# worxli/ORB_SLAM

Hardware: AMD Instinct MI355X
Metric: frames/sec ORB extract+match (640x480, 1000 kp) (higher is better)
Workload: dtype u8

## Files before the change

### orb_slam_amd/__init__.py

```python
import ctypes
import os
from pathlib import Path

import numpy as np

_PKG = Path(__file__).resolve().parent
LIB_PATH = Path(os.environ.get("ORBX_LIBRARY", _PKG / "liborbx.so"))

ORBX_OK = 0
ERRORS = {-1: "ORBX_ERR_ARG", -2: "ORBX_ERR_HIP", -3: "ORBX_ERR_CAPACITY",
          -4: "ORBX_ERR_UNSUPPORTED", -5: "ORBX_ERR_NOMEM", -6: "ORBX_ERR_NOT_POSDEF"}

KEYPOINT = np.dtype([("x", "<f4"), ("y", "<f4"), ("size", "<f4"), ("angle", "<f4"),
                     ("response", "<f4"), ("octave", "<i4"), ("class_id", "<i4")])
assert KEYPOINT.itemsize == 28


class OrbxError(RuntimeError):
    def __init__(self, code, where):
        super().__init__(f"{where}: {ERRORS.get(code, code)}")
        self.code = code


class FrameView(ctypes.Structure):
# ... 505 lines not shown
        "orbx_dev_search_by_projection_frame_kf": ([vp, i, vp, i, vp, vp, vp, vp, vp, f, i, i, vp, i, ip], i),
        "orbx_dev_search_by_sim3": ([vp, i, vp, i, vp, vp, vp, vp, vp, vp, vp, vp, f, vp, vp, f, vp, vp, i, ip], i),
        "orbx_search_by_sim3": ([vp, vp, vp, vp, vp, vp, vp, vp, vp, vp, f, vp, vp, f, vp, vp, ip], i),
        "orbx_distinctive_descriptors": ([vp, i, vp, vp, vp], i),
        "orbx_search_by_projection_kf_sim3": ([vp, vp, vp, vp, vp, vp, i, vp, ip], i),
        "orbx_search_by_projection_frame_kf": ([vp, vp, vp, vp, vp, vp, vp, vp, f, i, i, vp, ip], i),
        "orbx_vocab_create": ([vp, i, i, i, vp, vp, vp, vp, ctypes.POINTER(vp)], i),
        "orbx_vocab_destroy": ([vp], None),
        "orbx_vocab_n_words": ([vp], i),
        "orbx_vocab_transform": ([vp, vp, i, vp, i, vp, vp, vp, vp, vp, ip, vp, vp, vp, ip], i),
        "orbx_dev_compute_bow": ([vp, vp, i, i, i], i),
        "orbx_dev_read_bow": ([vp, i, i, vp, vp, vp, vp, vp, ip, vp, vp, vp, ip], i),
        "orbx_dev_search_by_bow": ([vp, i, i, vp, f, i, vp, i, vp], i),
        "orbx_dev_search_by_bow_kf": ([vp, i, vp, i, vp, vp, f, i, vp, i, vp], i),
        "orbx_dev_search_for_triangulation": ([vp, i, vp, i, vp, vp, vp, vp, i, i, vp, i, vp], i),
        "orbx_undistort_keypoints": ([vp, i, vp, vp, vp, vp], i),
        "orbx_compute_image_bounds": ([i, i, vp, vp, vp], i),
        "orbx_dev_undistort": ([vp, i, i, vp, vp], i),
        "orbx_pose_optimization": ([vp, vp, ip, vp], i),
        "orbx_pose_optimization_batch": ([vp, i, vp, vp, vp], i),
        "orbx_pose_stage": ([vp, i, vp], i),
        "orbx_pose_run": ([vp], i),
        "orbx_pose_fetch": ([vp, vp, vp, vp], i),
        "orbx_version": ([], ctypes.c_char_p),
        "orbx_abi_version": ([], i),
        "orbx_lba_set_workgroups": ([vp, i], i),
        "orbx_lba_get_workgroups": ([vp], i),
        "orbx_lba_last_workgroups": ([vp], i),
        "orbx_debug_lba_split": ([vp, i, i, i, i], i),
        "orbx_debug_describe_patch": ([vp, i, i, i, i, vp], i),
        "orbx_debug_level0_direct": ([vp], i),
        "orbx_debug_fast_instance": ([vp, vp], i),
        "orbx_debug_fast_lists": ([vp, i, vp, i, vp, i, vp], i),
        "orbx_pose_set_exact": ([vp, i], i),
        "orbx_pose_get_exact": ([vp], i),
        "orbx_dev_set_image_bounds": ([vp, vp], i),
        "orbx_set_launch_mode": ([vp, i], i),
        "orbx_get_launch_mode": ([vp], i),
        "orbx_host_alloc": ([sz, ctypes.POINTER(vp)], i),
        "orbx_host_free": ([vp], None),
        "orbx_dev_upload_async": ([vp, i, i, vp, i, i, sz], i),
        "orbx_dev_download_async": ([vp, i, i, vp, vp, vp, vp, vp], i),
        "orbx_describe_levels": ([i, f, i, i, i, i, vp, i], i),
        "orbx_init_models": ([vp, vp], i),
        "orbx_init_models_batch": ([vp, i, vp], i),
        "orbx_dev_init_models": ([vp, i, i, i, f, i, vp], i),
        "orbx_dev_read_init_models": ([vp, i, vp], i),
        "orbx_init_reconstruct": ([vp, vp], i),
        "orbx_init_reconstruct_batch": ([vp, i, vp], i),
        "orbx_dev_init_reconstruct": ([vp, i, i, i, vp, f, f, i], i),
        "orbx_dev_read_init_reconstruct": ([vp, i, vp, ip], i),
        "orbx_triangulate_matches": ([vp, vp, i, vp, i, vp, vp, vp, vp, vp, vp, vp, vp], i),
        "orbx_create_new_map_points": ([vp, vp, vp, i, vp, vp, vp, i, i, vp, vp, vp, vp, vp, vp], i),
        "orbx_dev_create_new_map_points": ([vp, i, vp, vp, i, vp, vp, vp, vp, i, i, vp, vp, vp, vp, vp, vp, i], i),
        "orbx_sim3_ransac": ([vp, vp], i),
        "orbx_sim3_ransac_batch": ([vp, i, vp], i),
        "orbx_pnp_ransac": ([vp, vp], i),
        "orbx_pnp_ransac_batch": ([vp, i, vp], i),
        "orbx_dev_pnp_candidates": ([vp, i, i, vp, vp, vp, vp, i, f, i, i, vp, i, vp, vp, vp], i),
        "orbx_dev_sim3_candidates": ([vp, i, vp, i, vp, vp, f, i, i, ctypes.c_double, i, i, i, vp, vp, i, vp, vp, vp], i),
        "orbx_optimize_sim3": ([vp, vp], i),
        "orbx_optimize_sim3_batch": ([vp, i, vp], i),
        "orbx_dev_optimize_sim3": ([vp, i, vp, vp, i, vp, vp, vp], i),
    }
    for name, (args, res) in sigs.items():
        fn = getattr(L, name)
# ... 144 lines not shown
                                            ctypes.byref(n)), "orbx_dev_read_features")
        return kps[:n.value].copy(), desc[:n.value].copy()

    def matches(self, slot):
        m = np.zeros(self.nfeatures, np.int32)
        nm, n1 = ctypes.c_int(0), ctypes.c_int(0)
        _check(lib().orbx_dev_read_matches(self._h, slot, _ptr(m), self.nfeatures, ctypes.byref(nm),
                                           ctypes.byref(n1)), "orbx_dev_read_matches")
        return m, nm.value

    def level(self, slot, level, blurred=False, cap=4 << 20):
        buf = np.zeros(cap, np.uint8)
        pw, ph = ctypes.c_int(0), ctypes.c_int(0)
        _check(lib().orbx_dev_read_level(self._h, slot, level, int(blurred), _ptr(buf), cap,
                                         ctypes.byref(pw), ctypes.byref(ph)), "orbx_dev_read_level")
        return buf[:pw.value * ph.value].reshape(ph.value, pw.value).copy()

    def describe_patch(self, slot, level, x, y):
        out = np.zeros((37, 37), np.uint8)
        _check(lib().orbx_debug_describe_patch(self._h, slot, level, x, y, _ptr(out)), "orbx_debug_describe_patch")
        return out

    def level0_direct(self):
        r = lib().orbx_debug_level0_direct(self._h)
        if r < 0:
            raise OrbxError(r, "orbx_debug_level0_direct")
        return bool(r)

    def fast_instance(self):
        out = np.zeros(3, np.int32)
        _check(lib().orbx_debug_fast_instance(self._h, _ptr(out)), "orbx_debug_fast_instance")
        return tuple(int(v) for v in out)

    def fast_lists(self, slot, cells_cap=1 << 14, lists_cap=1 << 22):
        cells = np.zeros(10 * cells_cap, np.int32)
        lists = np.zeros(lists_cap, np.uint32)
        ne = ctypes.c_int(0)
        n = lib().orbx_debug_fast_lists(self._h, slot, _ptr(cells), cells.size, _ptr(lists), lists.size,
                                        ctypes.byref(ne))
        _check(min(n, 0), "orbx_debug_fast_lists")
        out = []
        for level, ini_x, ini_y, hx, hy, valid, off, cap, cnt, _ in cells[:10 * n].reshape(n, 10):
            assert 0 <= cnt <= cap and off + cnt <= ne.value, (cnt, cap, off, ne.value)
            e = lists[off:off + cnt]
            xy = np.stack([e & 0xFFF, (e >> 12) & 0xFFF, e >> 24], axis=1).astype(np.int64)
            out.append((int(level), int(ini_x), int(ini_y), int(hx), int(hy), bool(valid), xy))
        return out

    def timing(self, enable=True, only=None):
        _check(lib().orbx_dev_kernel_time_select(self._h, only.encode() if only else None), "timing")
        _check(lib().orbx_dev_kernel_time_enable(self._h, int(enable)), "timing")

    def kernel_time(self, name):
        avg, tot = ctypes.c_double(0), ctypes.c_double(0)
        n = lib().orbx_dev_kernel_time(self._h, name.encode(), ctypes.byref(avg), ctypes.byref(tot))
        if n < 0:
            raise OrbxError(n, "orbx_dev_kernel_time")
        return n, avg.value, tot.value

    def pose_optimization(self, frames):
        from .synth_pose import PoseStats
        arr = (type(frames[0]) * len(frames))(*frames)
        n = np.zeros(len(frames), np.int32)
        st = (PoseStats * len(frames))()
        _check(lib().orbx_pose_optimization_batch(self._h, len(frames), arr, _ptr(n), st),
               "orbx_pose_optimization_batch")
# ... 356 lines not shown
```

### orb_slam_amd/csrc/orbx_api.cpp

```cpp
#include <cstdlib>
#include <algorithm>
#include <cstring>
#include <new>

#include "orbx_internal.h"

using namespace orbx;

namespace orbx {

static KernelTimer* find_timer(orbx_ctx* ctx, const char* name)
{
    for (auto& t : ctx->timers)
        if (t.name == name) return &t;
    ctx->timers.push_back(KernelTimer{name, {}, {}, 0});
    return &ctx->timers.back();
}

void timer_begin(orbx_ctx* ctx, const char* name, hipStream_t st)
{
    if (!ctx->timing || (!ctx->timing_only.empty() && ctx->timing_only != name)) return;
    KernelTimer* t = find_timer(ctx, name);
    if (t->used == (int)t->start.size()) {
        hipEvent_t a, b;
// ... 21 lines not shown
    ctx->scratch_bytes = 0;
    if (hipMalloc(&ctx->scratch, bytes) != hipSuccess) return ORBX_ERR_NOMEM;
    ctx->scratch_bytes = bytes;
    return ORBX_OK;
}

int ensure_pinned(orbx_ctx* ctx, size_t bytes)
{
    if (bytes <= ctx->host_pinned_bytes) return ORBX_OK;
    if (ctx->host_pinned) hipHostFree(ctx->host_pinned);
    ctx->host_pinned = nullptr;
    ctx->host_pinned_bytes = 0;
    if (hipHostMalloc(&ctx->host_pinned, bytes, hipHostMallocDefault) != hipSuccess) return ORBX_ERR_NOMEM;
    ctx->host_pinned_bytes = bytes;
    return ORBX_OK;
}

template <typename T>
static int realloc_dev(T*& p, size_t count)
{
    if (p) (void)hipFree(p);
    p = nullptr;
    if (count == 0) count = 1;
    if (hipMalloc(reinterpret_cast<void**>(&p), count * sizeof(T)) != hipSuccess) return ORBX_ERR_NOMEM;
    return ORBX_OK;
}

static void free_buffers(orbx_ctx* ctx)
{
    void* ptrs[] = {ctx->frames, ctx->pyr_raw, ctx->pyr_blur, ctx->cell_lists, ctx->retain_scratch, ctx->cell_count,
                    ctx->level_keys, ctx->cell_keys64, ctx->level_keys64, ctx->level_count, ctx->out_kps, ctx->out_desc, ctx->out_n,
                    ctx->match12, ctx->match_n, ctx->error_flags, ctx->dgeom.levels, ctx->dgeom.cells,
                    ctx->dgeom.res_cols, ctx->dgeom.res_rows, ctx->dgeom.umax, ctx->blur_tiles, ctx->cascade,
                    ctx->scratch, ctx->pose_dev, ctx->bow_dev};
    for (void* p : ptrs)
        if (p) (void)hipFree(p);
    if (ctx->host_pinned) (void)hipHostFree(ctx->host_pinned);
    if (ctx->pose_host) (void)hipHostFree(ctx->pose_host);
}

static int set_geometry(orbx_ctx* ctx, int w, int h)
{
    if (ctx->geom_w == w && ctx->geom_h == h) return ORBX_OK;
    if (w > ctx->max_w || h > ctx->max_h) return ORBX_ERR_CAPACITY;
    hipStreamSynchronize(ctx->stream);
    Geometry& g = ctx->geom;
    int r = compute_geometry(g, w, h);
    if (r != ORBX_OK) return r;
    plan_cascade(g, kCascadeLds);
    const int S = ctx->slots;
    if ((long long)w * h > (long long)ctx->cap_frame_px) {
        if ((r = realloc_dev(ctx->frames, (size_t)S * w * h)) != ORBX_OK) return r;
        ctx->cap_frame_px = (long long)w * h;
    }
    if (g.frame_pyr_bytes > ctx->cap_pyr_bytes) {
        if ((r = realloc_dev(ctx->pyr_raw, (size_t)S * g.frame_pyr_bytes)) != ORBX_OK) return r;
        if ((r = realloc_dev(ctx->pyr_blur, (size_t)g.frame_pyr_bytes)) != ORBX_OK) return r;
        ctx->cap_pyr_bytes = g.frame_pyr_bytes;
    }
    if (g.list_entries + 4LL * (long long)g.cells.size() > ctx->cap_list_entries) {
        const long long e = g.list_entries + 4LL * (long long)g.cells.size();
        if ((r = realloc_dev(ctx->cell_lists, (size_t)S * e)) != ORBX_OK) return r;
        if ((r = realloc_dev(ctx->retain_scratch, (size_t)S * e)) != ORBX_OK) return r;
        if (ctx->harris && (r = realloc_dev(ctx->cell_keys64, (size_t)S * e)) != ORBX_OK) return r;
        ctx->cap_list_entries = e;
    }
    if ((int)g.cells.size() > ctx->cap_cells) {
        if ((r = realloc_dev(ctx->cell_count, (size_t)S * g.cells.size())) != ORBX_OK) return r;
        if ((r = realloc_dev(ctx->dgeom.cells, g.cells.size())) != ORBX_OK) return r;
        ctx->cap_cells = (int)g.cells.size();
    }
    if (g.level_entries > ctx->cap_level_entries) {
        if ((r = realloc_dev(ctx->level_keys, (size_t)S * g.level_entries)) != ORBX_OK) return r;
        if (ctx->harris && (r = realloc_dev(ctx->level_keys64, (size_t)S * g.level_entries)) != ORBX_OK) return r;
        ctx->cap_level_entries = g.level_entries;
    }
    if ((int)g.res_cols.size() > ctx->cap_res_cols) {
        if ((r = realloc_dev(ctx->dgeom.res_cols, g.res_cols.size())) != ORBX_OK) return r;
        ctx->cap_res_cols = (int)g.res_cols.size();
    }
    if ((int)g.res_rows.size() > ctx->cap_res_rows) {
        if ((r = realloc_dev(ctx->dgeom.res_rows, g.res_rows.size())) != ORBX_OK) return r;
        ctx->cap_res_rows = (int)g.res_rows.size();
    }
    std::vector<int4> tiles;
    for (int l = 0; l < g.nlevels; l++) {
        const LevelGeom& L = g.levels[l];
        const int ndw = L.stride / 4, nstrips = (L.ph + kBlurStrip - 1) / kBlurStrip;
        const int nchunks = (ndw + kBlurChunkCols - 1) / kBlurChunkCols;
        for (int b = 0; b < nchunks * nstrips; b += kBlurItems / 64) tiles.push_back(make_int4(l, b, nchunks, nstrips));
    }
    if ((int)tiles.size() > ctx->cap_blur_tiles) {
        if ((r = realloc_dev(ctx->blur_tiles, tiles.size())) != ORBX_OK) return r;
        ctx->cap_blur_tiles = (int)tiles.size();
    }
    ctx->blur_tiles_n = (int)tiles.size();
    ORBX_HIP_CHECK(hipMemcpy(ctx->dgeom.levels, g.levels.data(), g.levels.size() * sizeof(LevelGeom), hipMemcpyHostToDevice));
    ORBX_HIP_CHECK(hipMemcpy(ctx->dgeom.cells, g.cells.data(), g.cells.size() * sizeof(CellGeom), hipMemcpyHostToDevice));
    if (!g.res_cols.empty())
        ORBX_HIP_CHECK(hipMemcpy(ctx->dgeom.res_cols, g.res_cols.data(), g.res_cols.size() * sizeof(ResizeCol), hipMemcpyHostToDevice));
    if (!g.res_rows.empty())
// ... 659 lines not shown
```

### orb_slam_amd/csrc/orbx_extract.hip

```cpp
#include <algorithm>
#include <type_traits>

#include "orbx_device.h"
#include "orbx_internal.h"

namespace orbx {

constexpr size_t kRetainLds = 128 * 1024;
constexpr int kRetainCellCap = 512;
constexpr int kSplitMinFrames = 16;
constexpr size_t kResizeLds = 96 * 1024;

__constant__ __attribute__((aligned(4))) int8_t c_pattern[256][4] = {
#include "orbx_pattern.inc"
};

#ifdef ORBX_FAST_PROFILE
__device__ unsigned long long g_fast_prof[24];
__device__ inline unsigned long long fp_stamp()
{
    unsigned long long t;
    asm volatile("s_memtime %0\n\ts_waitcnt lgkmcnt(0)" : "=s"(t)::"memory");
    return t;
}
#define FP_T0() unsigned long long _ft = fp_stamp()
#define FP_MARK(k)                                                                  \
    do {                                                                            \
        const unsigned long long _n = fp_stamp();                                   \
        if (threadIdx.x == 0) atomicAdd(&g_fast_prof[k], _n - _ft);                 \
        _ft = _n;                                                                   \
    } while (0)
#define FP_ADD(k, v) atomicAdd(&g_fast_prof[k], (unsigned long long)(v))
extern "C" int orbx_debug_fast_prof(unsigned long long* out)
{
    return hipMemcpyFromSymbol(out, HIP_SYMBOL(g_fast_prof), sizeof(unsigned long long) * 24) == hipSuccess ? 0 : -2;
}
#else
#define FP_T0()
#define FP_MARK(k)
#define FP_ADD(k, v)
#endif

struct ExtractArgs {
    const LevelGeom* levels;
    const CellGeom* cells;
    const ResizeCol* res_cols;
    const ResizeRow* res_rows;
    const int* umax;
    const uint8_t* frames;
    uint8_t* pyr_raw;
    uint8_t* pyr_blur;
    uint32_t* cell_lists;
    int32_t* cell_count;
    uint32_t* level_keys;
    int32_t* level_count;
    orbx_keypoint* out_kps;
    uint8_t* out_desc;
    int32_t* out_n;
    int32_t* error_flags;
    uint8_t* host_out;
    int32_t* retain_scratch;
    uint64_t* cell_keys64;
    uint64_t* level_keys64;
    int harris;
    int fp_contract;
    int nth_pivot;
    long long frame_pyr_bytes;
    int first_slot;
    int w, h;
    int nlevels, ncells, list_entries, level_entries, nfeatures;
    int fast_th, fast_th_low;
    int max_list_cap, max_level_cap;
    int l0_direct;
};

struct LevelSrc {
    const uint8_t* base;
    int stride;
};
static_assert(kEdge % 16 == 0, "the direct level 0 keeps the padded level's 16-byte alignment");
__device__ __forceinline__ LevelSrc level_src(const ExtractArgs& a, int f, int level, long long off, int stride)
{
    if (a.l0_direct && level == 0)
        return {a.frames + ((long long)(a.first_slot + f) * a.w * a.h - (long long)kEdge * a.w - kEdge), a.w};
    return {a.pyr_raw + (size_t)f * a.frame_pyr_bytes + off, stride};
}
// ... 612 lines not shown
                       __builtin_elementwise_minimum(e0, e9));
    }
    orbx_h2 dk = h2_max3(m[0], m[1], m[2]), br = h2_min3(x[0], x[1], x[2]);
    dk = h2_max3(dk, m[3], m[4]);
    br = h2_min3(br, x[3], x[4]);
    dk = h2_max3(dk, m[5], m[6]);
    br = h2_min3(br, x[5], x[6]);
    dk = __builtin_elementwise_maximum(dk, m[7]);
    br = __builtin_elementwise_minimum(br, x[7]);
    return __builtin_bit_cast(uint32_t, __builtin_elementwise_maximum(dk, -br));
}

__device__ inline int byte_of(uint32_t w, int k) { return (int)((w >> (8 * k)) & 0xFF); }

typedef short orbx_s16x2 __attribute__((ext_vector_type(2)));
__device__ inline uint32_t pk_sub16(uint32_t a, uint32_t b)
{
    return __builtin_bit_cast(uint32_t, (orbx_s16x2)(__builtin_bit_cast(orbx_s16x2, a) - __builtin_bit_cast(orbx_s16x2, b)));
}
__device__ inline uint32_t pk_max16(uint32_t a, uint32_t b)
{
    return __builtin_bit_cast(uint32_t,
                              __builtin_elementwise_max(__builtin_bit_cast(orbx_s16x2, a), __builtin_bit_cast(orbx_s16x2, b)));
}
__device__ inline orbx_h2 h2_bytes(uint32_t w, uint32_t k64, uint32_t sel)
{
    return __builtin_bit_cast(orbx_h2, __builtin_amdgcn_perm(k64, w, sel));
}

constexpr int kFastWideThreads = 256;
__host__ __device__ constexpr int fast_tile_bytes(int hy_max, int pitch) { return (hy_max * pitch + 511) & ~511; }
__host__ __device__ constexpr int fast_lds_bytes(int tile_bytes) { return 2 * tile_bytes + tile_bytes / 32; }
__host__ __device__ constexpr int fast_static_lds(bool u32_entries) { return 4 * 384 * (u32_entries ? 4 : 2) + 64; }
#ifndef ORBX_FAST_LDS_TARGET
#define ORBX_FAST_LDS_TARGET (40 * 1024)
#endif
constexpr int kFastLdsTarget = ORBX_FAST_LDS_TARGET;
#ifndef ORBX_DIAG_REPEAT
#define ORBX_DIAG_REPEAT 1, 1, 1, 1
#endif
constexpr int kDiagRepeat[4] = {ORBX_DIAG_REPEAT};

template <int kP, int kThreads = 256, bool kBanded = false>
__global__ __launch_bounds__(kThreads) __attribute__((amdgpu_waves_per_eu(kThreads > 256 ? 6 : 4))) void k_fast_cells(
    ExtractArgs a, int tile_bytes, int band_rows)
{
    constexpr int kBlock = kThreads, kWaves = kThreads / 64;
    extern __shared__ __attribute__((aligned(16))) uint8_t smem[];
    __shared__ BlockScratchN<kWaves> bs;
    using QEntry = typename std::conditional<kP != 0, uint16_t, uint32_t>::type;
    constexpr int kQueue = 128 + 256;
    constexpr int kQueueWords = kWaves * kQueue * (int)sizeof(QEntry) / 4;
    constexpr int kUnitCap = 2 * kQueueWords;
    __shared__ __attribute__((aligned(16))) uint32_t qbuf[kQueueWords];
    __shared__ int s_left[kWaves];
    uint16_t* ulist = reinterpret_cast<uint16_t*>(qbuf);
    const int f = blockIdx.y, tid = threadIdx.x, lane = tid & 63, wv = tid >> 6;
    QEntry* cand = reinterpret_cast<QEntry*>(qbuf) + wv * kQueue;
    const int clear16 = (tile_bytes + tile_bytes / 32) >> 4;
    auto clear_maps_at = [&](uint8_t* sm) {
        for (int i = tid; i < clear16; i += kBlock) reinterpret_cast<uint4*>(sm)[i] = make_uint4(0, 0, 0, 0);
    };
    auto process = [&](const int cell, uint8_t* const tile, uint8_t* const sm) {
    const CellGeom C = cget(a.cells, cell);
    int32_t* count_out = a.cell_count + (size_t)f * a.ncells + cell;
    if (!C.valid) {
        if (tid == 0) *count_out = 0;
        return;
    }
    const LevelGeom L = cget(a.levels, C.level);
    const int roi_x = kEdge + C.ini_x, x_al = roi_x & ~15, sh = roi_x - x_al;
    const int hx = C.hx, hy = C.hy;
    const int nq16 = (sh + hx + 15) >> 4;
    const int P = kP ? kP : 16 * nq16, nq = P >> 2;
    const LevelSrc ls = level_src(a, f, C.level, L.off, L.stride);
    const int lstride = ls.stride;
    const uint8_t* src = ls.base + (size_t)(kEdge + C.ini_y) * lstride + x_al;
    uint32_t* tile32 = reinterpret_cast<uint32_t*>(tile);
    uint32_t* sm32 = reinterpret_cast<uint32_t*>(sm);
    uint32_t* kept = tile32;
    uint32_t* nz = reinterpret_cast<uint32_t*>(sm + tile_bytes);
    FP_T0();
    auto load_tile = [&](int w0, int wh) {
        uint4* t16 = reinterpret_cast<uint4*>(tile32);
        const uint8_t* src_w = src + (size_t)w0 * lstride;
        const int n = wh * nq16;
        const float inv16 = 1.0f / (float)nq16;
        auto row_of = [&](int i) { return (int)(((float)i + 0.5f) * inv16); };
        for (int u0 = 0; u0 < n; u0 += 4 * kBlock) {
            const int i0 = min(u0 + tid, n - 1), i1 = min(u0 + kBlock + tid, n - 1);
            const int i2 = min(u0 + 2 * kBlock + tid, n - 1), i3 = min(u0 + 3 * kBlock + tid, n - 1);
            const int r0 = row_of(i0), r1 = row_of(i1), r2 = row_of(i2), r3 = row_of(i3);
            const int c0 = i0 - r0 * nq16, c1 = i1 - r1 * nq16, c2 = i2 - r2 * nq16, c3 = i3 - r3 * nq16;
            const uint4 v0 = *reinterpret_cast<const uint4*>(src_w + (uint32_t)(r0 * lstride + 16 * c0));
            const uint4 v1 = *reinterpret_cast<const uint4*>(src_w + (uint32_t)(r1 * lstride + 16 * c1));
            const uint4 v2 = *reinterpret_cast<const uint4*>(src_w + (uint32_t)(r2 * lstride + 16 * c2));
            const uint4 v3 = *reinterpret_cast<const uint4*>(src_w + (uint32_t)(r3 * lstride + 16 * c3));
            t16[r0 * (P >> 4) + c0] = v0;
            t16[r1 * (P >> 4) + c1] = v1;
            t16[r2 * (P >> 4) + c2] = v2;
            t16[r3 * (P >> 4) + c3] = v3;
        }
    };
    auto clear_maps = [&]() { clear_maps_at(sm); };
    auto clear_kept = [&]() {
        for (int i = tid; i < (tile_bytes >> 7); i += kBlock) reinterpret_cast<uint4*>(kept)[i] = make_uint4(0, 0, 0, 0);
    };
    const int c_lo = 3 + sh, c_hi = hx - 4 + sh;
    const int q0 = c_lo >> 2, nqe = c_hi >= c_lo ? (c_hi >> 2) - q0 + 1 : 0;
    const int j_lo = c_lo & 3, j_hi = c_hi & 3;
    const uint32_t k64 = 0x64646464u;
    auto score_pass = [&](const int tmin, const int sr0, const int nrows) {
        const int nunits = max(nrows, 0) * nqe;
        if (nunits <= 0) return;
        auto set_nz = [&](int p) { atomicOr(&nz[p >> 7], 1u << ((p >> 2) & 31)); };
        auto score_pair = [&](int pa, int pb, bool has_a, bool has_b) {
            if (!has_a) return;
            const uint32_t rb = fast_arc2(tile, pa, pb, P);
            const int Sa = (int)(int16_t)rb - 1, Sb = ((int32_t)rb >> 16) - 1;
            if (Sa >= tmin) {
                sm[pa] = (uint8_t)Sa;
                set_nz(pa);
            }
            if (has_b && Sb >= tmin) {
                sm[pb] = (uint8_t)Sb;
                set_nz(pb);
            }
        };
        const orbx_h2 T1 = {(_Float16)(tmin + 1), (_Float16)(tmin + 1)};
        auto cut_mask = [](bool c) {
            const uint32_t m = __builtin_amdgcn_readfirstlane(c ? ~0u : 0u);
            uint64_t r = ((uint64_t)m << 32) | m;
            asm("" : "+s"(r));
            return r;
        };
        const uint64_t cutA0 = cut_mask(j_lo > 0), cutA1 = cut_mask(j_lo > 1), cutA2 = cut_mask(j_lo > 2);
        const uint64_t cutB1 = cut_mask(j_hi < 1), cutB2 = cut_mask(j_hi < 2), cutB3 = cut_mask(j_hi < 3);
        typedef __attribute__((address_space(3))) QEntry LdsEntry;
        const uint32_t cand_lds = __builtin_amdgcn_readfirstlane((uint32_t)(uintptr_t)(LdsEntry*)cand);
        constexpr int kEsh = sizeof(QEntry) == 2 ? 1 : 2;
        uint32_t qe = cand_lds;
        auto compass = [&](const int pos, const int qr, const uint64_t live) {
            const uint32_t* row = reinterpret_cast<const uint32_t*>(tile + pos);
            const uint32_t mid = row[0];
            const uint32_t lo = row[-1], hi = row[1];
            const uint32_t up = row[-3 * nq], dn = row[3 * nq];
            const uint32_t p4w = __builtin_amdgcn_alignbyte(hi, mid, 3);
            const uint32_t p12w = __builtin_amdgcn_alignbyte(mid, lo, 1);
            uint32_t xw[2];
#pragma unroll
            for (int hf = 0; hf < 2; hf++) {
                const uint32_t sel = hf ? 0x04030401u : 0x04020400u;
                const orbx_h2 v = h2_bytes(mid, k64, sel);
                const orbx_h2 p0 = h2_bytes(dn, k64, sel), p4 = h2_bytes(p4w, k64, sel);
                const orbx_h2 p8 = h2_bytes(up, k64, sel), p12 = h2_bytes(p12w, k64, sel);
                const orbx_h2 A = __builtin_elementwise_maximum(__builtin_elementwise_minimum(p4, p12),
                                                                __builtin_elementwise_minimum(p0, p8));
                const orbx_h2 B = __builtin_elementwise_minimum(__builtin_elementwise_maximum(p4, p12),
                                                                __builtin_elementwise_maximum(p0, p8));
// ... 145 lines not shown
            if (bits) atomicOr(&kept[idx >> 3], bits << (4 * (idx & 7)));
        };
        const int nw = (wh * nq + 31) >> 5;
        const int pw = (nw + kBlock - 1) / kBlock;
        const int w0 = min(tid * pw, nw), w1 = min(w0 + pw, nw);
        int cnt = 0;
        for (int w = w0; w < w1; w++) cnt += __popc(nz[w]);
        int total;
        const int off0 = block_exclusive_scan(cnt, &total, bs, 1);
        for (int base = 0; base < total; base += kUnitCap) {
            if (base > 0) __syncthreads();
            if (cnt && off0 < base + kUnitCap && off0 + cnt > base) {
                int off = off0;
                for (int w = w0; w < w1; w++) {
                    uint32_t b = nz[w];
                    while (b) {
                        const int bit = __builtin_ctz(b);
                        b &= b - 1;
                        if (off >= base && off < base + kUnitCap) ulist[off - base] = (uint16_t)(32 * w + bit);
                        off++;
                    }
                }
            }
            __syncthreads();
            const int n = min(total - base, kUnitCap);
#ifdef ORBX_FAST_PROFILE
            if (tid == 0) FP_ADD(16, n);
            if (tid == 0) FP_ADD(17, (n + kBlock - 1) / kBlock);
#endif
            for (int i = tid; i < n; i += kBlock) nms_unit((int)ulist[i]);
        }
        return c1;
    };
    uint32_t* out = a.cell_lists + (size_t)f * a.list_entries + C.list_off;
    auto compact = [&](const int t, const int tmin, const int w0, const int wh, const int out_base) {
        const int nkw = (wh * P + 31) >> 5;
        const int per = (nkw + kBlock - 1) / kBlock;
        const int ka = min(tid * per, nkw), kb = min(ka + per, nkw);
        const bool all_kept = t == tmin;
#ifdef ORBX_FAST_PROFILE
        if (tid == 0) FP_ADD(18, per);
#endif
        int cnt = 0;
        for (int k = ka; k < kb; k++) {
            uint32_t b = kept[k];
            if (all_kept) {
                cnt += __popc(b);
            } else {
                while (b) {
                    const int bit = __builtin_ctz(b);
                    b &= b - 1;
                    cnt += sm[32 * k + bit] >= t;
                }
            }
        }
        int total;
        int off = out_base + block_exclusive_scan(cnt, &total, bs, 1);
        if (cnt) {
            for (int k = ka; k < kb; k++) {
                uint32_t b = kept[k];
                while (b) {
                    const int bit = __builtin_ctz(b);
                    b &= b - 1;
                    const int pos = 32 * k + bit;
                    const int s = sm[pos];
                    if (s >= t) {
                        if (off < C.list_cap) {
                            const int r = w0 + pos / P, cc = pos % P - sh;
                            out[off] = ((uint32_t)s << 24) | ((uint32_t)(C.ini_y + r) << 12) | (uint32_t)(C.ini_x + cc);
                        }
                        off++;
                    }
                }
            }
        }
        return total;
    };
    auto band = [&](const int b0, const int b1, const int tmin, const bool loaded = false) {
        const int w0 = max(0, b0 - 4), wh = min(hy, b1 + 4) - w0;
        const int s0 = max(3, b0 - 1), s1 = min(hy - 4, b1);
        if (!loaded) {
            FP_MARK(7);
            load_tile(w0, wh);
            FP_MARK(5);
            clear_maps();
            FP_MARK(6);
            __syncthreads();
        }
        FP_MARK(0);
        score_pass(tmin, s0 - w0, s1 - s0 + 1);
        __syncthreads();
        FP_MARK(1);
        clear_kept();
        __syncthreads();
        const int n1 = block_sum(nms_pass(b0 - w0, b1 - w0, wh), bs, 0);
        __syncthreads();
        return n1;
    };
    int n1 = 0, written = 0;
    if constexpr (kBanded) {
        const int brows = band_rows > 0 ? band_rows : hy;
        for (int b0 = 3; b0 < hy - 3; b0 += brows) {
            const int b1 = min(b0 + brows, hy - 3);
            n1 += band(b0, b1, a.fast_th);
            written += compact(a.fast_th, a.fast_th, max(0, b0 - 4), min(hy, b1 + 4) - max(0, b0 - 4), written);
            __syncthreads();
        }
        if (n1 <= 3) {
            const int tmin2 = a.fast_th > a.fast_th_low ? a.fast_th_low : a.fast_th;
            written = 0;
            for (int b0 = 3; b0 < hy - 3; b0 += brows) {
                const int b1 = min(b0 + brows, hy - 3);
                band(b0, b1, tmin2);
                written += compact(a.fast_th_low, tmin2, max(0, b0 - 4), min(hy, b1 + 4) - max(0, b0 - 4), written);
                __syncthreads();
            }
        }
    } else if (hy > 6) {
        int tmin_final = a.fast_th;
        n1 = band(3, hy - 3, a.fast_th);
        FP_MARK(2);
        if (a.fast_th > a.fast_th_low && n1 <= 3) {
            if (threadIdx.x == 0) FP_ADD(8, 1);
            tmin_final = a.fast_th_low;
            band(3, hy - 3, a.fast_th_low);
            FP_MARK(3);
        }
        written = compact(n1 <= 3 ? a.fast_th_low : a.fast_th, tmin_final, 0, hy, 0);
    }
    if (tid == 0) {
        *count_out = written;
        if (written > C.list_cap) atomicOr(a.error_flags, 1);
    }
    FP_MARK(4);
    if (tid == 0) FP_ADD(9, 1);
    };
    process(blockIdx.x, smem, smem + tile_bytes);
}

__device__ inline void level_quota(const ExtractArgs& a, const LevelGeom& L, const int32_t* counts, int cell,
                                   int* keep_c, int* pre_c, int* level_total)
{
    const int lane = threadIdx.x & 63;
    const int nCells = L.n_cells, nfc = L.nfeatures_cell;
    constexpr int kPer = 4;
    int tot[kPer], ret[kPer];
    bool nomore[kPer];
    int toDist = 0, nNoMore = 0;
#pragma unroll
    for (int k = 0; k < kPer; k++) {
        const int c = lane + 64 * k;
        tot[k] = 0;
        ret[k] = 0;
        nomore[k] = false;
        if (64 * k < nCells && c < nCells) {
            tot[k] = counts[c];
            if (a.cells[L.cell_base + c].valid) {
                if (tot[k] > nfc) {
                    ret[k] = nfc;
                } else {
                    ret[k] = tot[k];
                    toDist += nfc - tot[k];
                    nomore[k] = true;
                    nNoMore++;
// ... 777 lines not shown
    const LevelGeom& L = ctx->geom.levels[level];
    if (x < kEdge || x >= L.w - kEdge || y < kEdge || y >= L.h - kEdge) return ORBX_ERR_ARG;
    ctx_enter(ctx);
    uint8_t* d = nullptr;
    if (hipDeviceSynchronize() != hipSuccess) return ORBX_ERR_HIP;
    if (hipMalloc(&d, kBrRows * kBrRows) != hipSuccess) return ORBX_ERR_NOMEM;
    const bool direct = level == 0 && kEdge == 16 && ctx->geom.w % 16 == 0;
    const long long fw = ctx->geom.w, fh = ctx->geom.h;
    const uint8_t* lev = direct ? ctx->frames + ((long long)slot * fw * fh - (long long)kEdge * fw - kEdge)
                                : ctx->pyr_raw + (size_t)slot * ctx->geom.frame_pyr_bytes + L.off;
    hipLaunchKernelGGL(k_debug_describe_patch, dim3(1), dim3(64), 0, ctx->stream, lev, direct ? (int)fw : L.stride,
                       direct ? 1 : 0, L, kEdge + x, kEdge + y, d);
    int r = ORBX_OK;
    if (hipStreamSynchronize(ctx->stream) != hipSuccess ||
        hipMemcpy(out, d, kBrRows * kBrRows, hipMemcpyDeviceToHost) != hipSuccess)
        r = ORBX_ERR_HIP;
    (void)hipFree(d);
    return r;
}

extern "C" int orbx_debug_level0_direct(orbx_ctx* ctx)
{
    if (!ctx) return ORBX_ERR_ARG;
    return ctx->last_l0_direct ? 1 : 0;
}

extern "C" int orbx_debug_fast_instance(orbx_ctx* ctx, int* out)
{
    if (!ctx || !out || ctx->last_fast[0] < 0) return ORBX_ERR_ARG;
    for (int k = 0; k < 3; k++) out[k] = ctx->last_fast[k];
    return ORBX_OK;
}

extern "C" int orbx_debug_fast_lists(orbx_ctx* ctx, int slot, int32_t* cells, int cells_cap, uint32_t* lists,
                                     int lists_cap, int* entries)
{
    using namespace orbx;
    if (!ctx || !cells || !lists || !entries || slot < 0 || slot >= ctx->slots) return ORBX_ERR_ARG;
    ctx_enter(ctx);
    const Geometry& g = ctx->geom;
    const int n = (int)g.cells.size();
    if (cells_cap < 10 * n || lists_cap < g.list_entries) return ORBX_ERR_CAPACITY;
    std::vector<int32_t> cnt(n);
    if (hipDeviceSynchronize() != hipSuccess ||
        hipMemcpy(cnt.data(), ctx->cell_count + (size_t)slot * n, 4 * (size_t)n, hipMemcpyDeviceToHost) != hipSuccess ||
        hipMemcpy(lists, ctx->cell_lists + (size_t)slot * g.list_entries, 4 * (size_t)g.list_entries,
                  hipMemcpyDeviceToHost) != hipSuccess)
        return ORBX_ERR_HIP;
    for (int c = 0; c < n; c++) {
        const CellGeom& C = g.cells[c];
        const int32_t v[10] = {C.level, C.ini_x, C.ini_y, C.hx, C.hy, C.valid ? 1 : 0, C.list_off, C.list_cap, cnt[c], 0};
        for (int k = 0; k < 10; k++) cells[10 * c + k] = v[k];
    }
    *entries = g.list_entries;
    return n;
}

namespace orbx {

int launch_extract(orbx_ctx* ctx, int first, int count, const MatchSpec* m)
{
    const Geometry& g = ctx->geom;
    if (count > 1 || (m && m->kind != 0 && ctx->async_match)) {
        const int r = ensure_aux_streams(ctx);
        if (r != ORBX_OK) return r;
    }
    for (int sl = first; sl < first + count && sl < (int)ctx->bow_ready.size(); sl++) ctx->bow_ready[sl] = 0;
    wait_uploads_overlap(ctx, first, count, ctx->stream);
    ExtractArgs a;
    a.levels = ctx->dgeom.levels;
    a.cells = ctx->dgeom.cells;
    a.res_cols = ctx->dgeom.res_cols;
    a.res_rows = ctx->dgeom.res_rows;
    a.umax = ctx->dgeom.umax;
    a.frames = ctx->frames;
    a.pyr_raw = ctx->pyr_raw + (size_t)first * g.frame_pyr_bytes;
    a.pyr_blur = nullptr;
    a.cell_lists = ctx->cell_lists + (size_t)first * g.list_entries;
    a.cell_count = ctx->cell_count + (size_t)first * g.cells.size();
    a.level_keys = ctx->level_keys + (size_t)first * g.level_entries;
    a.level_count = ctx->level_count + (size_t)first * g.nlevels;
    a.out_kps = ctx->out_kps;
    a.out_desc = ctx->out_desc;
    a.out_n = ctx->out_n;
    a.error_flags = ctx->error_flags;
    a.host_out = ctx->single_frame ? ctx->single_out : nullptr;
    a.retain_scratch = ctx->retain_scratch + (size_t)first * (g.list_entries + 4 * g.cells.size());
    a.harris = ctx->harris;
    a.fp_contract = ctx->fp_contract;
    a.nth_pivot = ctx->nth_pivot;
    if ((size_t)((ctx->harris ? 3 : 2) * g.max_level_cap + 8) * 4 > 160 * 1024) return ORBX_ERR_UNSUPPORTED;
    a.cell_keys64 = ctx->harris ? ctx->cell_keys64 + (size_t)first * g.list_entries : nullptr;
    a.level_keys64 = ctx->harris ? ctx->level_keys64 + (size_t)first * g.level_entries : nullptr;
    a.frame_pyr_bytes = g.frame_pyr_bytes;
    a.w = g.w;
    a.h = g.h;
    a.nlevels = g.nlevels;
    a.ncells = (int)g.cells.size();
    a.list_entries = g.list_entries;
    a.level_entries = g.level_entries;
    a.nfeatures = g.nfeatures;
    a.fast_th = min(max(g.fast_th, 0), 255);
    a.fast_th_low = 7;
    a.max_list_cap = g.max_list_cap;
    a.max_level_cap = g.max_level_cap;
    a.l0_direct = (kEdge == 16 && g.w % 16 == 0 && !(ctx->single_frame && g.cascade_bands > 0)) ? 1 : 0;
    ctx->last_l0_direct = a.l0_direct != 0;

    auto run_pyramid = [&](const ExtractArgs& x, int nb, hipStream_t st) {
        if (ctx->single_frame && g.cascade_bands > 0) {
            timer_begin(ctx, "resize", st);
            for (int rep = 0; rep < kDiagRepeat[0]; rep++) {
// ... 48 lines not shown
                const int items = (L.stride / 4) * ((L.ph + kPyrRows - 1) / kPyrRows);
                hipLaunchKernelGGL(k_pyr_resize, dim3((items + 255) / 256, nb), dim3(256), 0, st, x, l);
            }
            timer_end(ctx, "resize", st);
        }
    };
    auto run_rest = [&](const ExtractArgs& x, int nb, hipStream_t st, int parts) {
        if (parts & 1) {
        timer_begin(ctx, "fast", st);
        {
            int wmax = 0, hmax = 0;
            for (const CellGeom& c : g.cells) {
                if (!c.valid) continue;
                wmax = std::max(wmax, (15 + c.hx + 15) & ~15);
                hmax = std::max(hmax, c.hy);
            }
            const dim3 grid((int)g.cells.size(), nb);
            auto plan = [&](int P, int static_lds, int& band_rows) {
                band_rows = 0;
                const int whole = fast_tile_bytes(hmax, P);
                if (fast_lds_bytes(whole) + static_lds <= kFastLdsTarget || hmax <= 9) return whole;
                int wh = hmax;
                while (wh > 9 && fast_lds_bytes(fast_tile_bytes(wh, P)) + static_lds > kFastLdsTarget) wh--;
                const int nint = hmax - 6, bmax = wh - 8;
                const int nbands = (nint + bmax - 1) / bmax;
                band_rows = (nint + nbands - 1) / nbands;
                return fast_tile_bytes(std::min(hmax, band_rows + 8), P);
            };
            auto fast = [&](auto kern, int pitch, int bytes, int band_rows, int threads) {
                const int lds = fast_lds_bytes(bytes);
                ctx->last_fast[0] = pitch;
                ctx->last_fast[1] = threads;
                ctx->last_fast[2] = band_rows;
                hipLaunchKernelGGL(kern, grid, dim3(threads), lds, st, x, bytes, band_rows);
            };
            int br = 0, bytes = 0;
            auto fits = [&](int P) {
                if (wmax > P) return false;
                bytes = fast_tile_bytes(hmax, P);
                return bytes <= 65536;
            };
            auto fits_banded = [&](int P) {
                if (wmax > P) return false;
                bytes = plan(P, fast_static_lds(false), br);
                return bytes <= 65536;
            };
            if (fits(96)) fast(k_fast_cells<96>, 96, bytes, 0, 256);
            else if (fits(144)) {
                for (int rep = 0; rep < kDiagRepeat[3]; rep++) fast(k_fast_cells<144>, 144, bytes, 0, 256);
            } else if (fits(208)) fast(k_fast_cells<208>, 208, bytes, 0, 256);
            else if (fits_banded(336))
                fast(k_fast_cells<336, kFastWideThreads, true>, 336, bytes, br, kFastWideThreads);
            else {
                bytes = plan(wmax, fast_static_lds(true), br);
                fast(k_fast_cells<0, kFastWideThreads, true>, 0, bytes, br, kFastWideThreads);
            }
        }
        timer_end(ctx, "fast", st);
        }
        if (parts & 2) {
        timer_begin(ctx, "retain", st);
        {
            const int ew = x.harris ? 2 : 1;
            const int cw = (ew + 1) * kRetainCellCap + 8;
            const int cwaves = 4;
            const int lw = (ew + 1) * g.max_level_cap + 8;
            const int lwaves = 1;
// ... 143 lines not shown
```

### orb_slam_amd/csrc/orbx_internal.h

```cpp
#pragma once

#include <hip/hip_runtime.h>

#include <cstdint>
#include <memory>
#include <string>
#include <vector>

#include "../../include/orbx.h"

namespace orbx {

constexpr int kEdge = 16;
constexpr int kHalfPatch = 15;
constexpr int kPatch = 31;
constexpr int kMaxLevels = 16;
constexpr int kMaxFeatures = 4096;
constexpr int kGridCols = 64;
constexpr int kGridRows = 48;
#ifndef ORBX_BLUR_STRIP
#define ORBX_BLUR_STRIP 28
#endif
constexpr int kBlurStrip = ORBX_BLUR_STRIP;
constexpr int kBlurItems = 256;
// ... 156 lines not shown
    int max_w = 0, max_h = 0, slots = 0;
    int geom_w = -1, geom_h = -1;
    uint8_t* frames = nullptr;
    uint8_t* pyr_raw = nullptr;
    uint8_t* pyr_blur = nullptr;
    uint32_t* cell_lists = nullptr;
    int32_t* retain_scratch = nullptr;
    int32_t* cell_count = nullptr;
    uint32_t* level_keys = nullptr;
    uint64_t* cell_keys64 = nullptr;
    uint64_t* level_keys64 = nullptr;
    int harris = 0;
    int fp_contract = 0;
    int nth_pivot = ORBX_NTH_PIVOT_GCC48;
    int32_t* level_count = nullptr;
    orbx_keypoint* out_kps = nullptr;
    uint8_t* out_desc = nullptr;
    int32_t* out_n = nullptr;
    int32_t* match12 = nullptr;
    int32_t* match_n = nullptr;
    int32_t* error_flags = nullptr;
    long long cap_frame_px = 0;
    long long cap_pyr_bytes = 0;
    long long cap_list_entries = 0;
    long long cap_level_entries = 0;
    int cap_cells = 0;
    int cap_res_cols = 0, cap_res_rows = 0, cap_blur_tiles = 0;
    int4* blur_tiles = nullptr;
    int4* cascade = nullptr;
    int cap_cascade = 0;
    int blur_tiles_n = 0;
    int last_first = 0, last_count = 0;
    bool last_l0_direct = false;
    int last_fast[3] = {-1, 0, 0};
    int has_bounds = 0;
    float bounds[4] = {0.f, 0.f, 0.f, 0.f};
    void* scratch = nullptr;
    size_t scratch_bytes = 0;
    void* host_pinned = nullptr;
    size_t host_pinned_bytes = 0;
    orbx::LbaResident* lba_res = nullptr;
    int lba_workgroups = 0;
    void* lba_split = nullptr;
    size_t lba_split_bytes = 0;
    int lba_split_cap[2] = {0, 0};
    size_t lba_split_cap_lds[2] = {0, 0};
    int lba_last_workgroups = 0;
    bool lba_force_single = false;
    bool lba_split_timed_out = false;
    bool lba_split_fallback = true;
    int lba_split_coop = 0;
    int lba_dbg_fail = 0;
    int lba_dbg_cap = 0;
    int lba_res_iters[2] = {0, 0};
    void* pose_dev = nullptr;
    size_t pose_dev_bytes = 0;
    void* pose_host = nullptr;
    size_t pose_host_bytes = 0;
    bool pose_exact = true;
    int pose_wide_max = 1;
    int pose_P = 0;
    long long pose_E = 0;
    size_t pose_o_flags = 0, pose_o_out = 0, pose_out_bytes = 0;
    std::vector<int32_t> pose_edge_kp;
    std::vector<long long> pose_e0;
    bool pose_ran = false;
    void* bow_dev = nullptr;
// ... 104 lines not shown
```

Before: 311,400.

## Build sparse FAST candidate list in LDS to drive NMS and compaction

During FAST scoring, each wavefront ballots its candidates and appends their positions to an LDS list through a single wave-aggregated ds_add. When the list fits under the cap, NMS and output compaction walk only the listed candidates and never scan the full score map. When it overflows, the kernel falls back to the dense path, rebuilding the nonzero bitmap from the map. This is meant to cut full-tile scanning for sparse cells, at the cost of extra LDS, atomics, a per-cell path record and a new device buffer.

```diff
diff --git a/orb_slam_amd/__init__.py b/orb_slam_amd/__init__.py
--- a/orb_slam_amd/__init__.py
+++ b/orb_slam_amd/__init__.py
@@ -561,6 +561,8 @@
         "orbx_debug_level0_direct": ([vp], i),
         "orbx_debug_fast_instance": ([vp, vp], i),
         "orbx_debug_fast_lists": ([vp, i, vp, i, vp, i, vp], i),
+        "orbx_debug_fast_list_cap": ([vp, i], i),
+        "orbx_debug_fast_paths": ([vp, i, vp, i, vp], i),
         "orbx_pose_set_exact": ([vp, i], i),
         "orbx_pose_get_exact": ([vp], i),
         "orbx_dev_set_image_bounds": ([vp, vp], i),
@@ -771,6 +773,16 @@
         _check(lib().orbx_debug_fast_instance(self._h, _ptr(out)), "orbx_debug_fast_instance")
         return tuple(int(v) for v in out)
 
+    def set_fast_list_cap(self, n):
+        _check(lib().orbx_debug_fast_list_cap(self._h, int(n)), "orbx_debug_fast_list_cap")
+
+    def fast_paths(self, slot, cells_cap=1 << 14):
+        out = np.zeros(cells_cap, np.uint8)
+        cap = ctypes.c_int(0)
+        n = lib().orbx_debug_fast_paths(self._h, slot, _ptr(out), out.size, ctypes.byref(cap))
+        _check(min(n, 0), "orbx_debug_fast_paths")
+        return out[:n].copy(), cap.value
+
     def fast_lists(self, slot, cells_cap=1 << 14, lists_cap=1 << 22):
         cells = np.zeros(10 * cells_cap, np.int32)
         lists = np.zeros(lists_cap, np.uint32)
diff --git a/orb_slam_amd/csrc/orbx_api.cpp b/orb_slam_amd/csrc/orbx_api.cpp
--- a/orb_slam_amd/csrc/orbx_api.cpp
+++ b/orb_slam_amd/csrc/orbx_api.cpp
@@ -77,7 +77,7 @@
                     ctx->level_keys, ctx->cell_keys64, ctx->level_keys64, ctx->level_count, ctx->out_kps, ctx->out_desc, ctx->out_n,
                     ctx->match12, ctx->match_n, ctx->error_flags, ctx->dgeom.levels, ctx->dgeom.cells,
                     ctx->dgeom.res_cols, ctx->dgeom.res_rows, ctx->dgeom.umax, ctx->blur_tiles, ctx->cascade,
-                    ctx->scratch, ctx->pose_dev, ctx->bow_dev};
+                    ctx->scratch, ctx->pose_dev, ctx->bow_dev, ctx->fast_path};
     for (void* p : ptrs)
         if (p) (void)hipFree(p);
     if (ctx->host_pinned) (void)hipHostFree(ctx->host_pinned);
@@ -112,6 +112,7 @@
     }
     if ((int)g.cells.size() > ctx->cap_cells) {
         if ((r = realloc_dev(ctx->cell_count, (size_t)S * g.cells.size())) != ORBX_OK) return r;
+        if ((r = realloc_dev(ctx->fast_path, (size_t)S * g.cells.size())) != ORBX_OK) return r;
         if ((r = realloc_dev(ctx->dgeom.cells, g.cells.size())) != ORBX_OK) return r;
         ctx->cap_cells = (int)g.cells.size();
     }
diff --git a/orb_slam_amd/csrc/orbx_extract.hip b/orb_slam_amd/csrc/orbx_extract.hip
--- a/orb_slam_amd/csrc/orbx_extract.hip
+++ b/orb_slam_amd/csrc/orbx_extract.hip
@@ -16,7 +16,7 @@
 };
 
 #ifdef ORBX_FAST_PROFILE
-__device__ unsigned long long g_fast_prof[24];
+__device__ unsigned long long g_fast_prof[32];
 __device__ inline unsigned long long fp_stamp()
 {
     unsigned long long t;
@@ -33,7 +33,7 @@
 #define FP_ADD(k, v) atomicAdd(&g_fast_prof[k], (unsigned long long)(v))
 extern "C" int orbx_debug_fast_prof(unsigned long long* out)
 {
-    return hipMemcpyFromSymbol(out, HIP_SYMBOL(g_fast_prof), sizeof(unsigned long long) * 24) == hipSuccess ? 0 : -2;
+    return hipMemcpyFromSymbol(out, HIP_SYMBOL(g_fast_prof), sizeof(unsigned long long) * 32) == hipSuccess ? 0 : -2;
 }
 #else
 #define FP_T0()
@@ -52,6 +52,7 @@
     uint8_t* pyr_blur;
     uint32_t* cell_lists;
     int32_t* cell_count;
+    uint8_t* fast_path;
     uint32_t* level_keys;
     int32_t* level_count;
     orbx_keypoint* out_kps;
@@ -730,6 +731,11 @@
 __host__ __device__ constexpr int fast_tile_bytes(int hy_max, int pitch) { return (hy_max * pitch + 511) & ~511; }
 __host__ __device__ constexpr int fast_lds_bytes(int tile_bytes) { return 2 * tile_bytes + tile_bytes / 32; }
 __host__ __device__ constexpr int fast_static_lds(bool u32_entries) { return 4 * 384 * (u32_entries ? 4 : 2) + 64; }
+__host__ __device__ constexpr int fast_list_lds(int tile_bytes, int n, bool u32_entries)
+{
+    return n > 0 ? tile_bytes / 8 + (((n + 1) * (u32_entries ? 4 : 2) + 15) & ~15) : 0;
+}
+constexpr int kFastListCap = 1536;
 #ifndef ORBX_FAST_LDS_TARGET
 #define ORBX_FAST_LDS_TARGET (40 * 1024)
 #endif
@@ -741,7 +747,7 @@
 
 template <int kP, int kThreads = 256, bool kBanded = false>
 __global__ __launch_bounds__(kThreads) __attribute__((amdgpu_waves_per_eu(kThreads > 256 ? 6 : 4))) void k_fast_cells(
-    ExtractArgs a, int tile_bytes, int band_rows)
+    ExtractArgs a, int tile_bytes, int band_rows, int plist_cap)
 {
     constexpr int kBlock = kThreads, kWaves = kThreads / 64;
     extern __shared__ __attribute__((aligned(16))) uint8_t smem[];
@@ -755,7 +761,10 @@
     uint16_t* ulist = reinterpret_cast<uint16_t*>(qbuf);
     const int f = blockIdx.y, tid = threadIdx.x, lane = tid & 63, wv = tid >> 6;
     QEntry* cand = reinterpret_cast<QEntry*>(qbuf) + wv * kQueue;
-    const int clear16 = (tile_bytes + tile_bytes / 32) >> 4;
+    const int clear16 = (tile_bytes + tile_bytes / 32 + (plist_cap > 0 ? tile_bytes / 8 : 0)) >> 4;
+    uint16_t* kprefix = reinterpret_cast<uint16_t*>(qbuf);
+    int& s_nlist = bs.vars[0];
+    const uint32_t nlist_lds = (uint32_t)(uintptr_t)(__attribute__((address_space(3))) int*)&s_nlist;
     auto clear_maps_at = [&](uint8_t* sm) {
         for (int i = tid; i < clear16; i += kBlock) reinterpret_cast<uint4*>(sm)[i] = make_uint4(0, 0, 0, 0);
     };
@@ -776,8 +785,11 @@
     const uint8_t* src = ls.base + (size_t)(kEdge + C.ini_y) * lstride + x_al;
     uint32_t* tile32 = reinterpret_cast<uint32_t*>(tile);
     uint32_t* sm32 = reinterpret_cast<uint32_t*>(sm);
-    uint32_t* kept = tile32;
     uint32_t* nz = reinterpret_cast<uint32_t*>(sm + tile_bytes);
+    const bool listed = plist_cap > 0;
+    uint32_t* kept = listed ? nz + (tile_bytes >> 7) : tile32;
+    QEntry* plist = reinterpret_cast<QEntry*>(sm + tile_bytes + tile_bytes / 32 + tile_bytes / 8);
+    int path_mask = 0;
     FP_T0();
     auto load_tile = [&](int w0, int wh) {
         uint4* t16 = reinterpret_cast<uint4*>(tile32);
@@ -816,13 +828,46 @@
             if (!has_a) return;
             const uint32_t rb = fast_arc2(tile, pa, pb, P);
             const int Sa = (int)(int16_t)rb - 1, Sb = ((int32_t)rb >> 16) - 1;
-            if (Sa >= tmin) {
-                sm[pa] = (uint8_t)Sa;
-                set_nz(pa);
-            }
-            if (has_b && Sb >= tmin) {
-                sm[pb] = (uint8_t)Sb;
-                set_nz(pb);
+            const bool st_a = Sa >= tmin, st_b = has_b && Sb >= tmin;
+            if (listed) {
+                const uint64_t ma = __builtin_amdgcn_ballot_w64(st_a), mb = __builtin_amdgcn_ballot_w64(st_b);
+                const uint32_t na = (uint32_t)__popcll(ma), nab = na + (uint32_t)__popcll(mb);
+                uint32_t base = 0;
+                if (nab) {
+                    const uint32_t first = (uint32_t)__builtin_ctzll(ma | mb);
+                    uint64_t saved;
+                    uint32_t ret;
+                    asm volatile("s_mov_b64 %0, exec\n\t"
+                                 "s_mov_b64 exec, %2\n\tds_add_rtn_u32 %1, %3, %4\n\t"
+                                 "s_mov_b64 exec, %0\n\ts_waitcnt lgkmcnt(0)"
+                                 : "=&s"(saved), "=&v"(ret)
+                                 : "s"(1ull << first), "v"(nlist_lds), "v"(nab)
+                                 : "memory");
+                    base = (uint32_t)__builtin_amdgcn_readlane((int)ret, (int)first);
+#ifdef ORBX_FAST_PROFILE
+                    if (lane == first) FP_ADD(19, nab);
+#endif
+                }
+                const uint32_t ia = __builtin_amdgcn_mbcnt_hi((uint32_t)(ma >> 32), __builtin_amdgcn_mbcnt_lo((uint32_t)ma, base));
+                const uint32_t ib =
+                    __builtin_amdgcn_mbcnt_hi((uint32_t)(mb >> 32), __builtin_amdgcn_mbcnt_lo((uint32_t)mb, base + na));
+                if (st_a) {
+                    sm[pa] = (uint8_t)Sa;
+                    plist[min(ia, (uint32_t)plist_cap)] = (QEntry)pa;
+                }
+                if (st_b) {
+                    sm[pb] = (uint8_t)Sb;
+                    plist[min(ib, (uint32_t)plist_cap)] = (QEntry)pb;
+                }
+            } else {
+                if (st_a) {
+                    sm[pa] = (uint8_t)Sa;
+                    set_nz(pa);
+                }
+                if (st_b) {
+                    sm[pb] = (uint8_t)Sb;
+                    set_nz(pb);
+                }
             }
         };
         const orbx_h2 T1 = {(_Float16)(tmin + 1), (_Float16)(tmin + 1)};
@@ -1034,8 +1079,79 @@
         }
         return c1;
     };
+    bool on_list = false;
+    auto nms_list = [&](const int rb0, const int rb1, const int n) {
+        int c1 = 0;
+        const int ft = max(a.fast_th, 1);
+        for (int i = tid; i < n; i += kBlock) {
+            const int pos = (int)plist[i];
+            const uint8_t* m = sm + pos;
+            const uint32_t s = m[0];
+            const uint32_t up = max(max((uint32_t)m[-P - 1], (uint32_t)m[-P]), (uint32_t)m[-P + 1]);
+            const uint32_t dn = max(max((uint32_t)m[P - 1], (uint32_t)m[P]), (uint32_t)m[P + 1]);
+            bool keep = s > max(max(up, dn), max((uint32_t)m[-1], (uint32_t)m[1]));
+            if constexpr (kBanded) {
+                const int rw = pos / P;
+                keep = keep && rw >= rb0 && rw < rb1;
+            }
+            if (keep) {
+                atomicOr(&kept[pos >> 5], 1u << (pos & 31));
+                c1 += (int)s >= ft;
+            }
+        }
+#ifdef ORBX_FAST_PROFILE
+        if (tid == 0) FP_ADD(20, (n + kBlock - 1) / kBlock);
+        if (tid == 0) atomicMax(&g_fast_prof[21], (unsigned long long)n);
+#endif
+        return c1;
+    };
+    auto nz_from_map = [&]() {
+        for (int i = tid; i < (tile_bytes >> 2); i += kBlock) {
+            const uint64_t b = __builtin_amdgcn_ballot_w64(sm32[i] != 0);
+            if (lane == 0) *reinterpret_cast<uint64_t*>(&nz[i >> 5]) = b;
+        }
+    };
     uint32_t* out = a.cell_lists + (size_t)f * a.list_entries + C.list_off;
+    auto emit_list = [&](const int t, const int tmin, const int w0, const int wh, const int out_base) {
+        const int n = s_nlist;
+        if (t != tmin) {
+            for (int i = tid; i < n; i += kBlock) {
+                const int pos = (int)plist[i];
+                if (sm[pos] < t) atomicAnd(&kept[pos >> 5], ~(1u << (pos & 31)));
+            }
+            __syncthreads();
+        }
+        const int nkw = (wh * P + 31) >> 5;
+        const int per = (nkw + kBlock - 1) / kBlock;
+        const int ka = min(tid * per, nkw), kb = min(ka + per, nkw);
+        int cnt = 0;
+        for (int k = ka; k < kb; k++) cnt += __popc(kept[k]);
+        int total;
+        int off = block_exclusive_scan(cnt, &total, bs, 1);
+        for (int k = ka; k < kb; k++) {
+            kprefix[k] = (uint16_t)off;
+            off += __popc(kept[k]);
+        }
+        __syncthreads();
+        for (int i = tid; i < n; i += kBlock) {
+            const int pos = (int)plist[i];
+            const uint32_t w = kept[pos >> 5], bit = 1u << (pos & 31);
+            if (w & bit) {
+                const int o = out_base + (int)kprefix[pos >> 5] + __popc(w & (bit - 1));
+                if (o < C.list_cap) {
+                    const int r = w0 + pos / P, cc = pos % P - sh;
+                    out[o] = ((uint32_t)sm[pos] << 24) | ((uint32_t)(C.ini_y + r) << 12) | (uint32_t)(C.ini_x + cc);
+                }
+            }
+        }
+#ifdef ORBX_FAST_PROFILE
+        if (tid == 0) FP_ADD(22, total);
+        if (tid == 0) atomicMax(&g_fast_prof[23], (unsigned long long)total);
+#endif
+        return total;
+    };
     auto compact = [&](const int t, const int tmin, const int w0, const int wh, const int out_base) {
+        if (on_list) return emit_list(t, tmin, w0, wh, out_base);
         const int nkw = (wh * P + 31) >> 5;
         const int per = (nkw + kBlock - 1) / kBlock;
         const int ka = min(tid * per, nkw), kb = min(ka + per, nkw);
@@ -1086,6 +1202,7 @@
             load_tile(w0, wh);
             FP_MARK(5);
             clear_maps();
+            if (tid == 0) s_nlist = 0;
             FP_MARK(6);
             __syncthreads();
         }
@@ -1093,10 +1210,20 @@
         score_pass(tmin, s0 - w0, s1 - s0 + 1);
         __syncthreads();
         FP_MARK(1);
-        clear_kept();
-        __syncthreads();
-        const int n1 = block_sum(nms_pass(b0 - w0, b1 - w0, wh), bs, 0);
-        __syncthreads();
+        int c1;
+        on_list = listed && s_nlist <= plist_cap;
+        if (on_list) {
+            c1 = nms_list(b0 - w0, b1 - w0, s_nlist);
+        } else {
+            if (listed) nz_from_map();
+            else clear_kept();
+            __syncthreads();
+            c1 = nms_pass(b0 - w0, b1 - w0, wh);
+        }
+        path_mask |= on_list ? 1 : 2;
+        if (tid == 0) FP_ADD(on_list ? 24 : 25, 1);
+        const int n1 = block_sum(c1, bs, 0);
+        if (!on_list) __syncthreads();
         return n1;
     };
     int n1 = 0, written = 0;
@@ -1132,6 +1259,7 @@
     }
     if (tid == 0) {
         *count_out = written;
+        a.fast_path[(size_t)(a.first_slot + f) * a.ncells + cell] = (uint8_t)path_mask;
         if (written > C.list_cap) atomicOr(a.error_flags, 1);
     }
     FP_MARK(4);
@@ -1975,6 +2103,29 @@
     return ORBX_OK;
 }
 
+extern "C" int orbx_debug_fast_list_cap(orbx_ctx* ctx, int n)
+{
+    if (!ctx) return ORBX_ERR_ARG;
+    ctx->fast_list_cap = n < 0 ? -1 : n;
+    return ORBX_OK;
+}
+
+extern "C" int orbx_debug_fast_paths(orbx_ctx* ctx, int slot, uint8_t* out, int cap, int* list_cap)
+{
+    if (!ctx || !out || !list_cap || slot < 0 || slot >= ctx->slots || ctx->last_fast[0] < 0) return ORBX_ERR_ARG;
+    ctx_enter(ctx);
+    const orbx::Geometry& g = ctx->geom;
+    const int n = (int)g.cells.size();
+    if (cap < n) return ORBX_ERR_CAPACITY;
+    if (hipDeviceSynchronize() != hipSuccess ||
+        hipMemcpy(out, ctx->fast_path + (size_t)slot * n, (size_t)n, hipMemcpyDeviceToHost) != hipSuccess)
+        return ORBX_ERR_HIP;
+    for (int c = 0; c < n; c++)
+        if (!g.cells[c].valid) out[c] = 0;
+    *list_cap = ctx->last_fast[3];
+    return n;
+}
+
 extern "C" int orbx_debug_fast_lists(orbx_ctx* ctx, int slot, int32_t* cells, int cells_cap, uint32_t* lists,
                                      int lists_cap, int* entries)
 {
@@ -2021,6 +2172,7 @@
     a.pyr_blur = nullptr;
     a.cell_lists = ctx->cell_lists + (size_t)first * g.list_entries;
     a.cell_count = ctx->cell_count + (size_t)first * g.cells.size();
+    a.fast_path = ctx->fast_path;
     a.level_keys = ctx->level_keys + (size_t)first * g.level_entries;
     a.level_count = ctx->level_count + (size_t)first * g.nlevels;
     a.out_kps = ctx->out_kps;
@@ -2135,7 +2287,13 @@
                 ctx->last_fast[0] = pitch;
                 ctx->last_fast[1] = threads;
                 ctx->last_fast[2] = band_rows;
-                hipLaunchKernelGGL(kern, grid, dim3(threads), lds, st, x, bytes, band_rows);
+                const bool u32e = pitch == 0;
+                int cap = ctx->fast_list_cap < 0 ? kFastListCap : std::min(ctx->fast_list_cap, 4096);
+                if (cap > 0 && (lds + fast_static_lds(u32e) + fast_list_lds(bytes, cap, u32e) > kFastLdsTarget || bytes / 32 > 1536))
+                    cap = 0;
+                ctx->last_fast[3] = cap;
+                hipLaunchKernelGGL(kern, grid, dim3(threads), lds + fast_list_lds(bytes, cap, u32e), st, x, bytes, band_rows,
+                                   cap);
             };
             int br = 0, bytes = 0;
             auto fits = [&](int P) {
diff --git a/orb_slam_amd/csrc/orbx_internal.h b/orb_slam_amd/csrc/orbx_internal.h
--- a/orb_slam_amd/csrc/orbx_internal.h
+++ b/orb_slam_amd/csrc/orbx_internal.h
@@ -212,7 +212,9 @@
     int blur_tiles_n = 0;
     int last_first = 0, last_count = 0;
     bool last_l0_direct = false;
-    int last_fast[3] = {-1, 0, 0};
+    int last_fast[4] = {-1, 0, 0, 0};
+    int fast_list_cap = -1;
+    uint8_t* fast_path = nullptr;
     int has_bounds = 0;
     float bounds[4] = {0.f, 0.f, 0.f, 0.f};
     void* scratch = nullptr;
```

Measured after the change: 317,000 (median of 6 runs). 1.02x the previous value.
